# SJTMusicTeam/MusicGeneration

Measured on AMD Instinct MI355X. Metric: training events/sec (whole node), REMI seq_len=2048, higher is better.
Workload: dtype bf16; 1 GPU; cfg2 REMI_EventSeq MusicTransformer V=337 layers=6 d_model=512 seq_len=2048 bf16, fwd+smoothed-CE+bwd+Adam/Noam, dropout 0.2; global_batch=128, per_gpu_batch=128, seq_len=2048, parallelism=dp1, deterministic=True, streams=one stream, whole chip

## Files before the change

### musicgeneration_amd/csrc/rel_attn_bwd.hip

```cpp
#include <type_traits>
#include "rel_attn_common.hpp"

using namespace relattn;

#ifndef MGX_EXPERIMENTS
#define MGX_EXPERIMENTS 0
#endif
namespace {
constexpr int WAVES = 4;
}

__global__ __launch_bounds__(256) void attn_delta_kernel(const uint16_t* __restrict__ ctx,
                                                         const uint16_t* __restrict__ dctx, const float* __restrict__ lse,
                                                         float* __restrict__ delta, float* __restrict__ nlse2,
                                                         float* __restrict__ ndelta, int B, int L, int d) {
    const int heads = d >> 6;
    const long total = (long)B * L * heads * 8;
    const long gid = (long)blockIdx.x * blockDim.x + threadIdx.x;
    if (gid >= total) return;
    const int sub = (int)(gid & 7);
    const long grp = gid >> 3;
    const int i = (int)(grp % L);
    const int hd = (int)((grp / L) % heads);
    const long row = (grp / ((long)L * heads)) * L + i;
// ... 166 lines not shown
#pragma unroll
        for (int ks = 0; ks < 4; ++ks) c = mfma(frag_R(kt, a, hh, ks), qf[ks], c);
        if (MASKED) {
            if (dq == 0) {
#pragma unroll
                for (int r = 0; r < 16; ++r) c[r] = (crow(r, 0) > am) ? -INFINITY : c[r];
            }
            if (pw) {
                const uint32_t pwl = pw >> (4 * hh);
#pragma unroll
                for (int r = 0; r < 16; ++r) c[r] = (pwl & (1u << crow(r, 0))) ? -INFINITY : c[r];
            }
        }
#pragma unroll
        for (int r = 0; r < 16; ++r) c[r] = __builtin_amdgcn_exp2f(__builtin_fmaf(c[r], LOG2E, -lse2));
        f32x16 dp = zero16();
        const char* vt = smem + OFF_VR + cur * TILE_BYTES;
#pragma unroll
        for (int ks = 0; ks < 4; ++ks) dp = mfma(frag_R(vt, a, hh, ks), dof[ks], dp);
#pragma unroll
        for (int r = 0; r < 16; ++r) c[r] = c[r] * (dp[r] - dlt);
        bf16x8 df[2];
#pragma unroll
        for (int ss = 0; ss < 2; ++ss) {
            df[ss] = acc_to_frag(c, ss);
            dq0 = mfma(frag_T_onR(kt, lane, ss, 0), df[ss], dq0);
            dq1 = mfma(frag_T_onR(kt, lane, ss, 1), df[ss], dq1);
        }
#pragma unroll
        for (int ss = 0; ss < 2; ++ss) {
            const u32x4 wv = __builtin_bit_cast(u32x4, df[ss]);
#pragma unroll
            for (int j = 0; j < 4; ++j) {
                const int r0 = 8 * ss + 2 * j;
                *(uint16_t*)(dband + (p ? dwa1[r0] : dwa0[r0])) = (uint16_t)wv[j];
                *(uint16_t*)(dband + (p ? dwa1[r0 + 1] : dwa0[r0 + 1])) = (uint16_t)(wv[j] >> 16);
            }
        }
        wave_lds_fence();
#pragma unroll
        for (int ks = 0; ks < 2; ++ks) {
            const bf16x8 gq = *(const bf16x8*)(dband + a * DB_STRIDE + (p * 32 + 16 * ks + 8 * hh) * 2);
            dq0 = mfma(et[2 * ks], gq, dq0);
            dq1 = mfma(et[2 * ks + 1], gq, dq1);
        }
    };
    const int nmain = anypad ? 0 : Q0;
    auto main_step = [&](int s, auto par_tag) {
        constexpr int PAR = decltype(par_tag)::value;
        const int tn = min(s + 1, ntw - 1);
        const u32x4 kreg = k_tile(tn);
        const u32x4 vreg = v_tile(tn);
        const int dq = q0 - s;
        bf16x8 et[4];
#pragma unroll
        for (int ks = 0; ks < 2; ++ks) { et[2 * ks] = et_frag(dq, ks, 0); et[2 * ks + 1] = et_frag(dq, ks, 1); }
        f32x16 c = zero16();
#pragma unroll
        for (int ks = 0; ks < 4; ++ks) c = mfma(qf[ks], e[ks], c);
        band_put(c, PAR ^ 1);
        wave_lds_fence();
        c = band_get(PAR);
        wave_lds_fence();
#pragma unroll
        for (int ks = 0; ks < 4; ++ks) e[ks] = e_frag(dq - 2, ks);
        __builtin_amdgcn_sched_barrier(0x78F);
        tile_tail(c, dq, PAR, PAR, 0u, std::false_type{}, et);
        *(u32x4*)(smem + OFF_KR + (PAR ^ 1) * TILE_BYTES + st_offR) = kreg;
        *(u32x4*)(smem + OFF_VR + (PAR ^ 1) * TILE_BYTES + st_offR) = vreg;
        __syncthreads();
    };
    int s = 0;
    for (; s < nmain; s += 2) {
        main_step(s, std::integral_constant<int, 0>{});
        main_step(s + 1, std::integral_constant<int, 1>{});
    }

    for (; s < ntw; ++s) {
        const int cur = s & 1;
        const int tn = min(s + 1, ntw - 1);
        const u32x4 kreg = k_tile(tn);
        const u32x4 vreg = v_tile(tn);
        const int dq = q0 - s;
        if (dq >= 0) {
            const uint32_t pw = padword(s);
            bf16x8 et[4];
#pragma unroll
            for (int ks = 0; ks < 2; ++ks) { et[2 * ks] = et_frag(dq, ks, 0); et[2 * ks + 1] = et_frag(dq, ks, 1); }
            if (dq >= 1) {
                f32x16 qe = zero16();
#pragma unroll
                for (int ks = 0; ks < 4; ++ks) qe = mfma(qf[ks], e[ks], qe);
                band_put(qe, cur ^ 1);
            }
            wave_lds_fence();
            f32x16 c = band_get(cur);
            wave_lds_fence();
#pragma unroll
            for (int ks = 0; ks < 4; ++ks) e[ks] = e_frag(dq - 2, ks);
            tile_tail(c, dq, cur, cur, pw, std::true_type{}, et);
        }
        if (s + 1 < ntw) {
            *(u32x4*)(smem + OFF_KR + (cur ^ 1) * TILE_BYTES + st_offR) = kreg;
            *(u32x4*)(smem + OFF_VR + (cur ^ 1) * TILE_BYTES + st_offR) = vreg;
        }
        __syncthreads();
    }
    if (wave_on) store_rows_lds(dqkv + ((size_t)b * L + i0) * ld + hd * 64, ld, dq0, dq1, lane, 0.125f, smem + band_base);
}

#ifndef MGX_DQL_PEEL
#define MGX_DQL_PEEL 0
#endif
#ifndef MGX_DQL_KT
#define MGX_DQL_KT 1
#endif
namespace k1l {
constexpr int OFF_KR = 0;
constexpr int OFF_ET = OFF_KR + 2 * TILE_BYTES;
constexpr int XROW = 72;
constexpr int OFF_X = OFF_ET + 8 * 4096;
constexpr int DB_STRIDE = 144;
constexpr int OFF_DBAND = OFF_X + WAVES * 32 * XROW;
constexpr int LDS_BYTES = OFF_DBAND + WAVES * 32 * DB_STRIDE;
constexpr int DEPTH = 4;
}

__global__ __launch_bounds__(256, 2) void rel_attn_dq_lite_kernel(
    const uint16_t* __restrict__ qkv, const u32x4* __restrict__ EfT, const uint16_t* __restrict__ dst,
    uint16_t* __restrict__ dqkv, int L, int d, int bgroup) {
    using namespace k1l;
    extern __shared__ __attribute__((aligned(256))) char smem[];
    const int tid = threadIdx.x, lane = tid & 63;
    const int w = __builtin_amdgcn_readfirstlane(tid >> 6);
    const int a = lane & 31, hh = lane >> 5;
    const int heads = d >> 6;
    const int nqb = (L + 127) >> 7;
    const int b = (blockIdx.y / nqb) * bgroup + blockIdx.x / heads, hd = blockIdx.x % heads;
    const int qb = nqb - 1 - (blockIdx.y % nqb);
    const int I0 = qb * 128, Q0 = I0 >> 5;
    const int nchunk = L >> 5;
    const bool wave_on = I0 + w * 32 < L;
    const int q0 = wave_on ? Q0 + w : nchunk - 1;
    const int i0 = q0 * 32;
    const int ntw = min(Q0 + 4, nchunk);
    const size_t ld = (size_t)3 * d;
    const uint16_t* qkv_b = qkv + (size_t)b * L * ld;

    const int srow = tid >> 3, sch = tid & 7;
    const int st_offR = MGX_DQL_KT ? imgT_off(srow, sch) : imgR_off(srow, sch);
    const char* k_base = (const char*)(qkv_b + d + hd * 64);
    const uint32_t k_voff = (uint32_t)((srow * ld + sch * 8) * 2);
    const uint32_t tile_bytes = (uint32_t)(32 * ld * 2);
    auto k_tile = [&](int t) { return *(const u32x4*)(k_base + (size_t)min(t, ntw - 1) * tile_bytes + k_voff); };
    const uint32_t tid16 = (uint32_t)tid * 16u, lane16 = (uint32_t)lane * 16u;
    auto e_item = [&](int k) {
        return *(const u32x4*)((const char*)EfT + (size_t)min(max(Q0 - k, 0), nchunk - 1) * 4096 + tid16);
    };
    const size_t ntri = (size_t)nchunk * (nchunk + 1) / 2;
    const size_t row_tiles = ((size_t)b * heads + hd) * ntri + (size_t)q0 * (q0 + 1) / 2;
    const char* ds_row = (const char*)(dst + row_tiles * 1024);
    auto ds_load = [&](int J, int ss) {
        return __builtin_nontemporal_load((const u32x4*)(ds_row + (size_t)min(J, q0) * 2048 + ss * 1024 + lane16));
    };

    u32x4 dsr[DEPTH][2];
#pragma unroll
    for (int j = 0; j < DEPTH; ++j) { dsr[j][0] = ds_load(j, 0); dsr[j][1] = ds_load(j, 1); }
    *(u32x4*)(smem + OFF_KR + st_offR) = k_tile(0);
#pragma unroll
    for (int k = -3; k <= 0; ++k) *(u32x4*)(smem + OFF_ET + (k & 7) * 4096 + tid16) = e_item(k);
    u32x4 kq[2] = {k_tile(1), k_tile(2)}, eq[2] = {e_item(1), e_item(2)};
    for (int o = tid * 16; o < WAVES * 32 * DB_STRIDE; o += 256 * 16) *(u32x4*)(smem + OFF_DBAND + o) = u32x4{0, 0, 0, 0};
    __syncthreads();

    char* xt = smem + OFF_X + w * (32 * XROW);
    char* dband = smem + OFF_DBAND + w * (32 * DB_STRIDE);
    const int xw0 = a * XROW + 8 * hh;
    const int xi = lane & 15, xg = lane >> 4;
    const int xr0 = ((xi >> 2) + 4 * hh) * XROW + 32 * (xg & 1) + 8 * (xi & 3);
    int dwa0[16], dwa1[16];
#pragma unroll
    for (int r = 0; r < 16; ++r) {
        dwa0[r] = crow(r, hh) * DB_STRIDE + (((crow(r, hh) - a) & 63) << 1);
        dwa1[r] = crow(r, hh) * DB_STRIDE + (((crow(r, hh) - a + 32) & 63) << 1);
    }
    f32x16 dq0 = zero16(), dq1 = zero16();

    auto frag_X = [&](int s) {
        bf16x8 out;
#pragma unroll
        for (int jq = 0; jq < 2; ++jq) {
            const bf16x4 t4 = __builtin_amdgcn_ds_read_tr16_b64_v4bf16((lds_bf16x4_ptr)(xt + xr0 + (16 * s + 8 * jq) * XROW));
            out[4 * jq + 0] = t4[0]; out[4 * jq + 1] = t4[1]; out[4 * jq + 2] = t4[2]; out[4 * jq + 3] = t4[3];
        }
        return out;
    };
    auto compute = [&](int p, const char* kt, const char* ec, const u32x4 (&t)[2]) {
#pragma unroll
        for (int ss = 0; ss < 2; ++ss) {
            if (!(MGX_DQL_PEEL & 1)) {
                *(u32x2*)(xt + xw0 + 16 * (2 * ss)) = u32x2{t[ss].x, t[ss].y};
                *(u32x2*)(xt + xw0 + 16 * (2 * ss + 1)) = u32x2{t[ss].z, t[ss].w};
            }
#pragma unroll
            for (int j = 0; j < ((MGX_DQL_PEEL & 2) ? 1 : 4); ++j) {
                const int r0 = 8 * ss + 2 * j;
                *(uint16_t*)(dband + (p ? dwa1[r0] : dwa0[r0])) = (uint16_t)t[ss][j];
                *(uint16_t*)(dband + (p ? dwa1[r0 + 1] : dwa0[r0 + 1])) = (uint16_t)(t[ss][j] >> 16);
            }
        }
        wave_lds_fence();
#pragma unroll
        for (int ss = 0; ss < ((MGX_DQL_PEEL & 4) ? 1 : 2); ++ss) {
            const bf16x8 df = frag_X(ss);
            dq0 = mfma(MGX_DQL_KT ? frag_T(kt, lane, ss, 0) : frag_T_onR(kt, lane, ss, 0), df, dq0);
            dq1 = mfma(MGX_DQL_KT ? frag_T(kt, lane, ss, 1) : frag_T_onR(kt, lane, ss, 1), df, dq1);
        }
#pragma unroll
        for (int ks = 0; ks < ((MGX_DQL_PEEL & 8) ? 1 : 2); ++ks) {
            const bf16x8 gq = *(const bf16x8*)(dband + a * DB_STRIDE + (p * 32 + 16 * ks + 8 * hh) * 2);
            dq0 = mfma(*(const bf16x8*)(ec + (2 * ks) * 1024 + lane16), gq, dq0);
            dq1 = mfma(*(const bf16x8*)(ec + (2 * ks + 1) * 1024 + lane16), gq, dq1);
        }
        wave_lds_fence();
    };
    auto step = [&](int s, auto slot_tag, bool active) {
        constexpr int SLOT = decltype(slot_tag)::value, PAR = SLOT & 1;
        const u32x4 t[2] = {dsr[SLOT][0], dsr[SLOT][1]};
        dsr[SLOT][0] = ds_load(s + DEPTH, 0);
        dsr[SLOT][1] = ds_load(s + DEPTH, 1);
        if (active) compute(PAR, smem + OFF_KR + PAR * TILE_BYTES, smem + OFF_ET + ((s - w) & 7) * 4096, t);
        if (!(MGX_DQL_PEEL & 16)) {
            *(u32x4*)(smem + OFF_KR + (PAR ^ 1) * TILE_BYTES + st_offR) = kq[PAR];
            *(u32x4*)(smem + OFF_ET + ((s + 1) & 7) * 4096 + tid16) = eq[PAR];
            kq[PAR] = k_tile(s + 3);
            eq[PAR] = e_item(s + 3);
        }
        __syncthreads();
    };
    using S0_ = std::integral_constant<int, 0>; using S1_ = std::integral_constant<int, 1>;
    using S2_ = std::integral_constant<int, 2>; using S3_ = std::integral_constant<int, 3>;
    static_assert(DEPTH == 4, "the loops below are unrolled by DEPTH");
    __builtin_amdgcn_s_waitcnt(0x0F70);
    int s = 0;
    for (; s < Q0; s += 4) {
        step(s, S0_{}, true);
        step(s + 1, S1_{}, true);
        step(s + 2, S2_{}, true);
        step(s + 3, S3_{}, true);
    }
    step(s, S0_{}, q0 - s >= 0);
    if (s + 1 < ntw) step(s + 1, S1_{}, q0 - s - 1 >= 0);
    if (s + 2 < ntw) step(s + 2, S2_{}, q0 - s - 2 >= 0);
    if (s + 3 < ntw) step(s + 3, S3_{}, q0 - s - 3 >= 0);
    if (wave_on) store_rows_lds(dqkv + ((size_t)b * L + i0) * ld + hd * 64, ld, dq0, dq1, lane, 0.125f, dband);
}

#ifndef MGX_DKV_PEEL
#define MGX_DKV_PEEL 0
#endif
#ifdef MGX_DKV_STAMP
#define DKV_STAMP(i) do { __builtin_amdgcn_sched_barrier(0); const unsigned long long t_ = __builtin_amdgcn_s_memtime(); \
                          __builtin_amdgcn_sched_barrier(0); if (!MASKED) st_acc[i] += t_ - st_last; st_last = t_; } while (0)
#else
#define DKV_STAMP(i)
#endif
#ifndef MGX_DKV_IMGB
#define MGX_DKV_IMGB 0
#endif
#ifndef MGX_DKV_ONEIMG
#define MGX_DKV_ONEIMG 1
#endif
#ifndef MGX_DKV_WAVES
#define MGX_DKV_WAVES 4
#endif
#if 0
#endif
namespace k2 {
constexpr int KW = MGX_DKV_WAVES;
constexpr int OFF_QR = 0;
constexpr int OFF_QT = OFF_QR + 2 * TILE_BYTES;
constexpr int OFF_OR = OFF_QT + 2 * TILE_BYTES;
constexpr int OFF_OT = OFF_OR + 2 * TILE_BYTES;
constexpr int ST_BYTES = 256 * KW;
constexpr int OFF_ST = OFF_OT + 2 * TILE_BYTES;
constexpr int PATCH_BYTES = 4608;
constexpr int OFF_BAND = KW == 4 ? OFF_ST + 2 * ST_BYTES : 0;
constexpr int OFF_FLAG = KW == 4 ? OFF_BAND + KW * PATCH_BYTES : OFF_ST + 2 * ST_BYTES;
constexpr int LDS_BYTES = OFF_FLAG + 16;
}

template <bool EXPORT_DS>
__global__ __launch_bounds__(64 * k2::KW, 2) void rel_attn_dkv_kernel(
    const uint16_t* __restrict__ qkv, const u32x4* __restrict__ EfA, const uint32_t* __restrict__ padbits,
    const uint16_t* __restrict__ dctx, const float* __restrict__ nlse2 , const float* __restrict__ ndelta ,
    uint16_t* __restrict__ dqkv, uint16_t* __restrict__ dst, int L, int d, int bgroup) {
    using namespace k2;
    extern __shared__ __attribute__((aligned(256))) char smem[];
    const int tid = threadIdx.x, lane = tid & 63;
    const int w = __builtin_amdgcn_readfirstlane(tid >> 6);
    const int bl = lane & 31, hh = lane >> 5;
    const int heads = d >> 6;
    const int nkb = (L + 32 * KW - 1) / (32 * KW);
#ifndef MGX_DKV_XCD
#define MGX_DKV_XCD 0
#endif
    int bh_l = blockIdx.x, kbr = blockIdx.y % nkb;
    if (MGX_DKV_XCD && (gridDim.x & 7) == 0) {
        const int r = kbr * gridDim.x + bh_l, per = gridDim.x >> 3, m = r >> 3;
        kbr = m / per;
        bh_l = (m % per) * 8 + (r & 7);
    }
    const int b = (blockIdx.y / nkb) * bgroup + bh_l / heads, hd = bh_l % heads;
    const int J0 = kbr * 32 * KW;
    const int nchunk = L >> 5;
    const int nT = (L - J0) >> 5;
    const bool wave_on = J0 + w * 32 < L;
    const int wk = wave_on ? w : nT - 1;
    const int j0 = J0 + wk * 32;
    const size_t ld = (size_t)3 * d;
    const uint16_t* qkv_b = qkv + (size_t)b * L * ld;
    const size_t stat_base = ((size_t)b * heads + hd) * L;

    constexpr int NS = 4 / KW;
    const char* q_base = (const char*)(qkv_b + (size_t)J0 * ld + hd * 64);
    const char* o_base = (const char*)(dctx + ((size_t)b * L + J0) * d + hd * 64);
    uint32_t q_voffR[NS], q_voffT[NS], o_voffR[NS], o_voffT[NS];
#pragma unroll
    for (int i = 0; i < NS; ++i) {
        const int slot = tid + 64 * KW * i, srow = slot >> 3, spc = slot & 7;
        const int lcR = spc ^ (MGX_DKV_IMGB ? imgB_swz(srow) : ((srow >> 1) & 7)), lcT = spc ^ (((srow >> 1) & 1) << 2);
        q_voffR[i] = (uint32_t)((srow * ld + lcR * 8) * 2); q_voffT[i] = (uint32_t)((srow * ld + lcT * 8) * 2);
        o_voffR[i] = (uint32_t)((srow * d + lcR * 8) * 2);  o_voffT[i] = (uint32_t)((srow * d + lcT * 8) * 2);
    }
    const uint32_t q_step = (uint32_t)(32 * ld * 2), o_step = (uint32_t)(32 * d * 2);
    const uint32_t lane16 = (uint32_t)lane * 16u;
    auto e_frag = [&](int q, int ks) {
        return __builtin_bit_cast(bf16x8, *(const u32x4*)((const char*)EfA + (size_t)min(max(q, 0), nchunk - 1) * 4096 + ks * 1024 + lane16));
    };
    const uint32_t st_voff = (uint32_t)(((lane & 32) ? (const char*)ndelta - (const char*)nlse2 : 0) + (lane & 31) * 4);
    const char* st_base = (const char*)(nlse2 + stat_base + J0);
    const uint32_t lds_w = lds_addr_of(smem) + w * 1024;
    auto stage = [&](int t, int buf) {
        const int tn = (MGX_DKV_PEEL & 16) ? 0 : min(t, nT - 1);
        const char* qb = q_base + (size_t)tn * q_step;
        const char* ob = o_base + (size_t)tn * o_step;
#pragma unroll
        for (int i = 0; i < NS; ++i) {
            const uint32_t dw = lds_w + KW * 1024 * i + buf * TILE_BYTES;
            dma16(qb, q_voffR[i], dw + OFF_QR);
            if (!MGX_DKV_ONEIMG) dma16(qb, q_voffT[i], dw + OFF_QT);
            dma16(ob, o_voffR[i], dw + OFF_OR);
            if (!MGX_DKV_ONEIMG) dma16(ob, o_voffT[i], dw + OFF_OT);
        }
        dma4(st_base + (size_t)tn * 128, st_voff, lds_addr_of(smem) + OFF_ST + buf * ST_BYTES + w * 256);
    };
    stage(0, 0);
    bf16x8 kf[4], vf[4], e[2][4];
    uint32_t padlane = 0;
    int wgpad = 0;
    {
        const uint16_t* kp = qkv_b + (size_t)(j0 + bl) * ld + d + hd * 64 + hh * 8;
#pragma unroll
        for (int ks = 0; ks < 4; ++ks) {
            kf[ks] = __builtin_bit_cast(bf16x8, *(const u32x4*)(kp + ks * 16));
            vf[ks] = __builtin_bit_cast(bf16x8, *(const u32x4*)(kp + d + ks * 16));
            e[0][ks] = e_frag(0, ks);
            e[1][ks] = e[0][ks];
        }
        if (padbits) {
            const uint32_t pwv = padbits[(size_t)b * nchunk + (j0 >> 5)];
            padlane = (pwv >> bl) & 1u;
            if (tid == 0) *(volatile uint32_t*)(smem + OFF_FLAG) = 0u;
            __syncthreads();
            if (pwv) *(volatile uint32_t*)(smem + OFF_FLAG) = 1u;
            __syncthreads();
            wgpad = __builtin_amdgcn_readfirstlane(*(volatile uint32_t*)(smem + OFF_FLAG));
        }
    }
    asm volatile("s_waitcnt vmcnt(0)" ::: "memory");
    __syncthreads();
    char* band = smem + OFF_BAND + w * PATCH_BYTES;
    uint32_t rd[16];
#pragma unroll
    for (int r = 0; r < 16; ++r) rd[r] = (uint32_t)((hh * 32 + ((crow(r, hh) - bl) & 31)) << 2);
    f32x16 dk0 = zero16(), dk1 = zero16(), dv0 = zero16(), dv1 = zero16();
    char* ds_col = nullptr;
    if (EXPORT_DS) {
        const size_t ntri = (size_t)nchunk * (nchunk + 1) / 2;
        ds_col = (char*)(dst + (((size_t)b * heads + hd) * ntri + (size_t)(j0 >> 5)) * 1024) + lane16;
    }
    auto ds_tile = [&](int t) {
        const size_t I = (size_t)(J0 >> 5) + t;
        return ds_col + (I * (I + 1) / 2) * 2048;
    };

#ifdef MGX_DKV_STAMP
    unsigned long long st_acc[6] = {0, 0, 0, 0, 0, 0}, st_last = 0;
    unsigned st_steps = 0;
    const unsigned long long st_t0 = __builtin_amdgcn_s_memtime(), st_r0 = __builtin_amdgcn_s_memrealtime();
#endif
    auto tile = [&](int dq, int cur, auto par_tag, auto masked_tag, char* dsp, int tnext) {
        constexpr int PAR = decltype(par_tag)::value;
        constexpr bool MASKED = decltype(masked_tag)::value;
        DKV_STAMP(5);
        const char* qr = smem + OFF_QR + cur * TILE_BYTES;
        bf16x8 qa[4];
// ... 224 lines not shown
            for (int ks = 0; ks < 4; ++ks) qa[ks] = frag_R(qr, bl, hh, ks);
            f32x16 qe = zero16();
#pragma unroll
            for (int ks = 0; ks < 4; ++ks) qe = mfma(qa[ks], ef[ks], qe);
#pragma unroll
            for (int r = 0; r < 16; ++r) *(float*)(band + (crow(r, hh) * 32 + bl) * 4) = qe[r];
            wave_lds_fence();
            f32x16 srel;
#pragma unroll
            for (int r = 0; r < 16; ++r) {
                const int ar = crow(r, hh);
                srel[r] = *(const float*)(band + (ar * 32 + ((ar - bl) & 31)) * 4);
            }
            const bool has_up = (u >= 1);
            const char* klo = smem + OFF_KR + (u % KV_SLOTS) * TILE_BYTES;
            const char* vlo = smem + OFF_VR + (u % KV_SLOTS) * TILE_BYTES;
            const char* kup = smem + OFF_KR + ((u + KV_SLOTS - 1) % KV_SLOTS) * TILE_BYTES;
            const char* vup = smem + OFF_VR + ((u + KV_SLOTS - 1) % KV_SLOTS) * TILE_BYTES;
            f32x16 slo = srel, sup = srel;
#pragma unroll
            for (int ks = 0; ks < 4; ++ks) slo = mfma(qa[ks], frag_R(klo, bl, hh, ks), slo);
            if (has_up) {
#pragma unroll
                for (int ks = 0; ks < 4; ++ks) sup = mfma(qa[ks], frag_R(kup, bl, hh, ks), sup);
            }
            bool plo = false, pup = !has_up;
            if (pb) {
                plo = (pb[u] >> bl) & 1u;
                if (has_up) pup = (pb[u - 1] >> bl) & 1u;
            }
            const char* orr = smem + OFF_OR + cur * TILE_BYTES;
            bf16x8 oa[4];
#pragma unroll
            for (int ks = 0; ks < 4; ++ks) oa[ks] = frag_R(orr, bl, hh, ks);
            f32x16 dlo = zero16(), dup = zero16();
#pragma unroll
            for (int ks = 0; ks < 4; ++ks) dlo = mfma(oa[ks], frag_R(vlo, bl, hh, ks), dlo);
            if (has_up) {
#pragma unroll
                for (int ks = 0; ks < 4; ++ks) dup = mfma(oa[ks], frag_R(vup, bl, hh, ks), dup);
            }
            const char* st = smem + OFF_ST + cur * 256;
            f32x16 ds;
#pragma unroll
            for (int g4 = 0; g4 < 4; ++g4) {
                const f32x4 l4 = (MGX_DKV_PEEL & 32) ? f32x4{9.f, 9.f, 9.f, 9.f} : *(const f32x4*)(st + (8 * g4 + 4 * hh) * 4);
                const f32x4 d4 = (MGX_DKV_PEEL & 32) ? f32x4{0.f, 0.f, 0.f, 0.f} : *(const f32x4*)(st + 128 + (8 * g4 + 4 * hh) * 4);
#pragma unroll
                for (int k = 0; k < 4; ++k) {
                    const int r = 4 * g4 + k;
                    const bool lower = (bl <= crow(r, hh));
                    const bool masked = lower ? plo : pup;
                    const float sv = lower ? slo[r] : sup[r];
                    const float dv = lower ? dlo[r] : dup[r];
                    const float p = masked ? 0.f : __builtin_amdgcn_exp2f(__builtin_fmaf(sv, LOG2E, -l4[k]));
                    ds[r] = p * (dv - d4[k]);
                }
            }
            wave_lds_fence();
#pragma unroll
            for (int r = 0; r < 16; ++r) {
                const int ar = crow(r, hh);
                *(float*)(band + (ar * 32 + ((ar - bl) & 31)) * 4) = ds[r];
            }
            wave_lds_fence();
            f32x16 x;
#pragma unroll
            for (int r = 0; r < 16; ++r) x[r] = *(const float*)(band + (crow(r, hh) * 32 + bl) * 4);
            wave_lds_fence();
            const char* qt = smem + OFF_QT + cur * TILE_BYTES;
#pragma unroll
            for (int ss = 0; ss < 2; ++ss) {
                const bf16x8 xf = acc_to_frag(x, ss);
                de0 = mfma(xf, frag_T(qt, lane, ss, 0), de0);
                de1 = mfma(xf, frag_T(qt, lane, ss, 1), de1);
            }
        }
        if (have_next) {
            *(u32x4*)(smem + (half ? OFF_VR : OFF_KR) + ((t + 1) % KV_SLOTS) * TILE_BYTES + st_offR) = kreg;
            if (half == 0) {
                const u32x4 qq = scale8(qreg, 0.125f);
                *(u32x4*)(smem + OFF_QR + (cur ^ 1) * TILE_BYTES + st_offR) = qq;
                *(u32x4*)(smem + OFF_QT + (cur ^ 1) * TILE_BYTES + st_offT) = qq;
            } else {
                *(u32x4*)(smem + OFF_OR + (cur ^ 1) * TILE_BYTES + st_offR) = qreg;
            }
            if (tid < 64) *(float*)(smem + OFF_ST + (cur ^ 1) * 256 + tid * 4) = streg;
        }
        __syncthreads();
    }
    if (wave_on) {
#pragma unroll
        for (int r = 0; r < 16; ++r) {
            const int dl = 32 * cw + crow(r, hh);
            float* row = dEr + (size_t)(L - 1 - dl) * 64;
            atomicAdd(row + bl, de0[r]);
            atomicAdd(row + 32 + bl, de1[r]);
        }
    }
}

#ifndef MGX_DET_PEEL
#define MGX_DET_PEEL 0
#endif
namespace k3t {
#ifndef MGX_DET_STEPS
#define MGX_DET_STEPS 32
#endif
constexpr int DIAGS = 4, RS = 64, STEPS = MGX_DET_STEPS, NW = 5;
constexpr int AROW = 352;
constexpr int OFF_A = 0;
constexpr int OFF_Q = RS * AROW;
constexpr int LDS_BYTES = OFF_Q + 2 * TILE_BYTES;
constexpr int SLOTS = 2;
}

__global__ __launch_bounds__(320, 4) void rel_attn_de_tiles_kernel(
    const uint16_t* __restrict__ qkv, const uint16_t* __restrict__ dst, float* __restrict__ dEr ,
    int bgroup, int ngroups, int wg_per_group, int L, int d,
    long long* __restrict__ det ) {
    using namespace k3t;
    extern __shared__ __attribute__((aligned(16))) char smem[];
    const int tid = threadIdx.x, lane = tid & 63;
    const int w = __builtin_amdgcn_readfirstlane(tid >> 6);
    const int l31 = lane & 31, hh = lane >> 5;
    const int heads = d >> 6, nbh = bgroup * heads;
    const size_t ld = (size_t)3 * d;
    const int nchunk = L >> 5;
    int t = 0, first = 0, ns = 0;
    const bool dealt = ngroups > 0;
    const int xk = dealt ? (int)(blockIdx.x >> 3) : (int)blockIdx.x;
    const int grp = dealt ? (xk / wg_per_group) * 8 + (int)(blockIdx.x & 7) : xk / wg_per_group;
    {
        int rest = xk % wg_per_group;
        const int ntile = (nchunk + DIAGS - 1) / DIAGS;
        for (t = 0; t < ntile; ++t) {
            ns = (L - t * DIAGS * 32 + RS - 1) / RS;
            const int nwg = (nbh * ns + STEPS - 1) / STEPS;
            if (rest < nwg) break;
            rest -= nwg;
        }
        if (t == ntile) return;
        first = rest * STEPS;
    }
    const int total = nbh * ns;
    const int last = min(total, first + STEPS);
    const int c0 = t * DIAGS, d0 = c0 * 32;
    const size_t ntri = (size_t)nchunk * (nchunk + 1) / 2;
    const int qrow = tid >> 3, qch = tid & 7;
    const uint32_t lane16 = (uint32_t)lane * 16u;
    const int wm = w & 3;
    const int sc_lane = hh * 4 * (AROW + 2) - 2 * l31;
    u32x4 areg[SLOTS][2], qreg[2];
    bool a_ok[SLOTS], q_ok[2];
    auto load_tiles = [&](int g) {
        const int bhl = g / ns, i0 = d0 + (g - bhl * ns) * RS;
        const int bh = grp * nbh + bhl;
        const int bb = bh / heads, hd = bh - bb * heads;
        const int I0 = i0 >> 5;
        const char* tp = (const char*)(dst + (size_t)bh * ntri * 1024) + lane16;
#pragma unroll
        for (int k = 0; k < SLOTS; ++k) {
            const int I = I0 + k, J = I - c0 - wm;
            a_ok[k] = I < nchunk && J >= 0;
            const size_t Ic = (size_t)min(I, nchunk - 1), Jc = (size_t)max(J, 0);
            const char* p = tp + (Ic * (Ic + 1) / 2 + min(Jc, Ic)) * 2048;
            areg[k][0] = __builtin_nontemporal_load((const u32x4*)p);
            areg[k][1] = __builtin_nontemporal_load((const u32x4*)(p + 1024));
        }
        const uint16_t* qp = qkv + ((size_t)bb * L + ((MGX_DET_PEEL & 4) ? 0 : i0)) * ld + hd * 64 + (qch & 7) * 8;
#pragma unroll
        for (int i = 0; i < 2; ++i) {
            const int r = (qrow & 31) + 32 * i;
            q_ok[i] = i0 + r < L;
            qreg[i] = *(const u32x4*)(qp + (size_t)min(r, L - 1 - i0) * ld);
        }
    };
    auto store_tiles = [&]() {
        const u32x4 zero = {0, 0, 0, 0};
        if (w < 4) {
#pragma unroll
            for (int k = 0; k < SLOTS; ++k) {
                char* base = smem + OFF_A + k * 32 * AROW + 64 * (wm + 1) + sc_lane;
#pragma unroll
                for (int ss = 0; ss < 2; ++ss) {
                    const u32x4 v = a_ok[k] ? areg[k][ss] : zero;
#pragma unroll
                    for (int j = 0; j < ((MGX_DET_PEEL & 1) ? 1 : 4); ++j) {
                        const int r0 = 8 * ss + 2 * j;
                        *(uint16_t*)(base + crow(r0, 0) * (AROW + 2)) = (uint16_t)v[j];
                        *(uint16_t*)(base + crow(r0 + 1, 0) * (AROW + 2)) = (uint16_t)(v[j] >> 16);
                    }
                }
            }
            char* qt = smem + OFF_Q;
#pragma unroll
            for (int i = 0; i < 2; ++i) {
                const int r = qrow + 32 * i;
                *(u32x4*)(qt + (r >> 5) * TILE_BYTES + imgT_off(r & 31, qch)) = q_ok[i] ? qreg[i] : zero;
            }
        }
    };
    f32x16 de0 = zero16(), de1 = zero16();
    const int fa_i = lane & 15, fa_g = lane >> 4;
    const int fa_off = (fa_i >> 2) * AROW + (32 * w) * 2 + (2 * (fa_g & 1) + ((fa_i & 3) >> 1)) * 16 + 8 * (fa_i & 1) + 8 * hh * AROW;
    auto multiply = [&]() {
        if (MGX_DET_PEEL & 2) return;
        const char* at = smem + OFF_A + fa_off;
        const char* qt = smem + OFF_Q;
#pragma unroll
        for (int ks = 0; ks < 4; ++ks) {
            bf16x8 af;
#pragma unroll
            for (int jq = 0; jq < 2; ++jq) {
                const bf16x4 tq = __builtin_amdgcn_ds_read_tr16_b64_v4bf16((lds_bf16x4_ptr)(at + (16 * ks + 4 * jq) * AROW));
                af[4 * jq + 0] = tq[0]; af[4 * jq + 1] = tq[1]; af[4 * jq + 2] = tq[2]; af[4 * jq + 3] = tq[3];
            }
            const char* qs = qt + (ks >> 1) * TILE_BYTES;
            de0 = mfma(af, frag_Tn(qs, lane, ks & 1, 0), de0);
            de1 = mfma(af, frag_Tn(qs, lane, ks & 1, 1), de1);
        }
    };
    for (int o = tid * 16; o < RS * AROW; o += NW * 64 * 16) *(u32x4*)(smem + OFF_A + o) = u32x4{0, 0, 0, 0};
    __syncthreads();
    if (first < last) {
        load_tiles(first);
        store_tiles();
    }
    __syncthreads();
    for (int g = first; g + 1 < last; ++g) {
        load_tiles(g + 1);
        __builtin_amdgcn_sched_barrier(0);
        multiply();
        __syncthreads();
        store_tiles();
        __syncthreads();
    }
    if (first < last) multiply();
#pragma unroll
    for (int r = 0; r < 16; ++r) {
        const int dl = d0 - 32 + 32 * w + crow(r, hh);
        if ((MGX_DET_PEEL & 8) && de0[r] + de1[r] != 12345.f) continue;
        if (dl >= 0 && dl < L) {
            if (det) {
                long long* drow = det + (size_t)(L - 1 - dl) * 64;
                det_add(drow + l31, 0.125f * de0[r]);
                det_add(drow + 32 + l31, 0.125f * de1[r]);
                continue;
            }
            float* row = dEr + (size_t)(L - 1 - dl) * 64;
            atomicAdd(row + l31, 0.125f * de0[r]);
            atomicAdd(row + 32 + l31, 0.125f * de1[r]);
        }
    }
}

static int bwd_batch_group(int B, int L, int d) {
    const double per_row = (double)L * d * 2 * 5;
    int g = B;
#if MGX_EXPERIMENTS
    static const int forced = [] { const char* e = getenv("MGX_ATTN_BGROUP"); return e ? atoi(e) : 0; }();
    if (forced > 0 && B % forced == 0) return forced;
#endif
    while (g > 1 && (g * per_row > 110e6 || B % g != 0)) --g;
    return g;
}

static size_t ws_stat_bytes(int B, int L, int d) { return (((size_t)B * (d / 64) * L * 4) + 255) / 256 * 256; }
static size_t ws_delta_bytes(int B, int L, int d) { return 3 * ws_stat_bytes(B, L, d); }

static size_t ws_ert_bytes(int L) { return 2 * er_frag_bytes(L); }

extern "C" size_t mgx_rel_attn_bwd_workspace(int B, int L, int d) {
    if (B <= 0 || L <= 0 || d <= 0) return 0;
    const size_t nchunk = (size_t)L / 32;
    return ws_delta_bytes(B, L, d) + ws_ert_bytes(L) + (size_t)B * (d / 64) * (nchunk * (nchunk + 1) / 2) * 2048;
}

extern "C" int mgx_rel_attn_bwd_parts(const uint16_t* qkv, const uint16_t* E, const uint32_t* padbits,
                                      const uint16_t* ctx, const uint16_t* dctx, const float* lse, uint16_t* dqkv,
                                      float* dE, void* workspace, size_t ws_bytes, int B, int L, int d, int M,
                                      int parts, void* stream) {
    MGX_REQUIRE(qkv && E && ctx && dctx && lse && dqkv && dE && workspace, MGX_ERR_NULL, "mgx_rel_attn_bwd: NULL pointer");
    MGX_REQUIRE(B > 0 && L > 0 && d > 0 && d % 64 == 0 && L % 32 == 0 && M >= L, MGX_ERR_SHAPE,
                "mgx_rel_attn_bwd: need d%%64==0, L%%32==0, M>=L (got B=%d L=%d d=%d M=%d)", B, L, d, M);
    MGX_REQUIRE(ws_bytes >= mgx_rel_attn_bwd_workspace(B, L, d) && ((uintptr_t)workspace & 255) == 0, MGX_ERR_SHAPE,
                "mgx_rel_attn_bwd: workspace must be 256-byte aligned and >= mgx_rel_attn_bwd_workspace() = %zu bytes (got %zu)",
                mgx_rel_attn_bwd_workspace(B, L, d), ws_bytes);
    MGX_REQUIRE(!((parts & 2) && (parts & 32)), MGX_ERR_SHAPE, "mgx_rel_attn_bwd: parts 2 and 32 both write dq");
    static const bool attr_once = [] {
        hipFuncSetAttribute((const void*)rel_attn_dq_kernel, hipFuncAttributeMaxDynamicSharedMemorySize, k1::LDS_BYTES);
        hipFuncSetAttribute((const void*)rel_attn_dq_lite_kernel, hipFuncAttributeMaxDynamicSharedMemorySize, k1l::LDS_BYTES);
        hipFuncSetAttribute((const void*)rel_attn_dkv_kernel<true>, hipFuncAttributeMaxDynamicSharedMemorySize, k2::LDS_BYTES);
        hipFuncSetAttribute((const void*)rel_attn_de_kernel, hipFuncAttributeMaxDynamicSharedMemorySize, k3::LDS_BYTES);
        hipFuncSetAttribute((const void*)rel_attn_de_tiles_kernel, hipFuncAttributeMaxDynamicSharedMemorySize, k3t::LDS_BYTES);
        return true;
    }();
    (void)attr_once;
    hipStream_t s = (hipStream_t)stream;
    const int heads = d / 64;
    const uint16_t* Er = E + (size_t)(M - L) * 64;
    float* delta = (float*)workspace;
    float* nlse2 = (float*)((char*)workspace + ws_stat_bytes(B, L, d));
    float* ndelta = (float*)((char*)workspace + 2 * ws_stat_bytes(B, L, d));
    u32x4* EfA = (u32x4*)((char*)workspace + ws_delta_bytes(B, L, d));
    u32x4* EfT = (u32x4*)((char*)EfA + er_frag_bytes(L));
    uint16_t* dst = (uint16_t*)((char*)EfA + ws_ert_bytes(L));
    if (parts & 1) {
        const long total = (long)B * L * heads * 8;
        hipLaunchKernelGGL(attn_delta_kernel, dim3((unsigned)((total + 255) / 256)), dim3(256), 0, s, ctx, dctx, lse, delta, nlse2, ndelta, B, L, d);
        launch_er_frag(Er, EfA, EfT, L, s);
    }
    const int bg = bwd_batch_group(B, L, d);
    MGX_REQUIRE((long)((L + 127) / 128) * (B / bg) <= 65535, MGX_ERR_SHAPE, "mgx_rel_attn_bwd: L/128 * batch groups too large");
    const dim3 gq(bg * heads, ((L + 127) / 128) * (B / bg));
    MGX_REQUIRE(!((parts & 4) && (parts & 64)), MGX_ERR_SHAPE, "mgx_rel_attn_bwd: parts 4 and 64 both write dk / dv and the dS tiles");
#ifndef MGX_DKV64_DEFAULT
#define MGX_DKV64_DEFAULT 1
#endif
    if ((parts & 4) && MGX_DKV64_DEFAULT && L % 128 == 0) {
        const int rc64 = dkv64_launch(qkv, EfA, padbits, dctx, nlse2, ndelta, dqkv, dst, B, L, d, bg, stream);
        if (rc64 != MGX_OK) return rc64;
    } else if (parts & (4 | 64)) {
#if MGX_EXPERIMENTS
        static const int dkv_lds = [] {
            const char* e = getenv("MGX_DKV_LDS");
            const int v = e ? atoi(e) : 0;
            if (v > k2::LDS_BYTES) hipFuncSetAttribute((const void*)rel_attn_dkv_kernel<true>, hipFuncAttributeMaxDynamicSharedMemorySize, v);
            return v > k2::LDS_BYTES ? v : k2::LDS_BYTES;
        }();
#else
        constexpr int dkv_lds = k2::LDS_BYTES;
#endif
        const dim3 gk(bg * heads, ((L + 32 * k2::KW - 1) / (32 * k2::KW)) * (B / bg));
        MGX_REQUIRE(gk.y <= 65535, MGX_ERR_SHAPE, "mgx_rel_attn_bwd: too many key blocks for the grid");
        hipLaunchKernelGGL(rel_attn_dkv_kernel<true>, gk, dim3(64 * k2::KW), dkv_lds, s, qkv, EfA, padbits, dctx, nlse2, ndelta, dqkv, dst, L, d, bg);
    }
    if (parts & 2)
        hipLaunchKernelGGL(rel_attn_dq_lite_kernel, gq, dim3(256), k1l::LDS_BYTES, s, qkv, EfT, dst, dqkv, L, d, bg);
    if (parts & 32)
        hipLaunchKernelGGL(rel_attn_dq_kernel, gq, dim3(256), k1::LDS_BYTES, s, qkv, EfA, EfT, padbits, dctx, lse, delta, dqkv, L, d, bg);
    if (parts & 8) {
#ifndef MGX_DET_BG
#define MGX_DET_BG 1
#endif
        const bool dealt = B % (8 * MGX_DET_BG) == 0;
        const int bgd = dealt ? MGX_DET_BG : bg, ngr = B / bgd;
        long nwg = 0;
        for (int t = 0; t < (L / 32 + k3t::DIAGS - 1) / k3t::DIAGS; ++t)
            nwg += ((long)bgd * heads * ((L - t * k3t::DIAGS * 32 + k3t::RS - 1) / k3t::RS) + k3t::STEPS - 1) / k3t::STEPS;
        const long grid = nwg * ngr;
        MGX_REQUIRE(grid < (1L << 31), MGX_ERR_SHAPE, "mgx_rel_attn_bwd: grid too large");
        int rc;
        long long* det = mgx_det_scratch((size_t)L * 64, stream, &rc);
        if (rc != MGX_OK) return rc;
        hipLaunchKernelGGL(rel_attn_de_tiles_kernel, dim3((unsigned)grid), dim3(64 * k3t::NW), k3t::LDS_BYTES, s, qkv, dst,
                           dE + (size_t)(M - L) * 64, bgd, dealt ? ngr : -ngr, (int)nwg, L, d, det);
        if (det) launch_det_fold(det, dE + (size_t)(M - L) * 64, (size_t)L * 64, 1.f, 1, s);
    }
    if (parts & 16) {
        const dim3 ge(B * heads, ((L >> 5) + k3::W3 - 1) / k3::W3);
        hipLaunchKernelGGL(rel_attn_de_kernel, ge, dim3(64 * k3::W3), k3::LDS_BYTES, s, qkv, Er, padbits, dctx, lse, delta,
                           dE + (size_t)(M - L) * 64, L, d);
    }
    MGX_CHECK_LAUNCH("mgx_rel_attn_bwd");
    return MGX_OK;
}

extern "C" int mgx_rel_attn_bwd(const uint16_t* qkv, const uint16_t* E, const uint32_t* padbits, const uint16_t* ctx,
                                const uint16_t* dctx, const float* lse, uint16_t* dqkv, float* dE, void* workspace,
                                size_t ws_bytes, int B, int L, int d, int M, void* stream) {
    return mgx_rel_attn_bwd_parts(qkv, E, padbits, ctx, dctx, lse, dqkv, dE, workspace, ws_bytes, B, L, d, M, 15, stream);
}
```

### musicgeneration_amd/csrc/rel_attn_common.hpp

```cpp
#pragma once
#include "mgx_common.hpp"

namespace relattn {

constexpr int DH = 64;
constexpr int TILE_BYTES = 32 * DH * 2;
constexpr float LOG2E = 1.4426950408889634f;
constexpr float PAD_NEG = -1.0e9f;

typedef __attribute__((address_space(3))) bf16x4* lds_bf16x4_ptr;
typedef __attribute__((address_space(3))) float* lds_f32_ptr;
typedef __attribute__((address_space(3))) char* lds_char_ptr;
MGX_DEV uint32_t lds_addr_of(const char* p) { return (uint32_t)(uintptr_t)(lds_char_ptr)p; }
MGX_DEV void lds_store_f32(uint32_t addr, float v) { *(lds_f32_ptr)(uintptr_t)addr = v; }

MGX_DEV int crow(int r, int hh) { return (r & 3) + 8 * (r >> 2) + 4 * hh; }

MGX_DEV int imgR_off(int row, int chunk) { return row * 128 + ((chunk ^ ((row >> 1) & 7)) << 4); }
MGX_DEV int imgT_off(int row, int chunk) { return row * 128 + ((chunk ^ (((row >> 1) & 1) << 2)) << 4); }

MGX_DEV bf16x8 frag_R(const char* tile, int row, int hh, int ks) {
    return *(const bf16x8*)(tile + imgR_off(row, 2 * ks + hh));
}

MGX_DEV bf16x8 frag_T(const char* tile, int lane, int s, int ct) {
    const int i = lane & 15, g = lane >> 4, hh = lane >> 5;
    const int rq = i >> 2;
    const int chunk = 4 * ct + 2 * (g & 1) + ((i & 3) >> 1);
    const int byte_in = 8 * (i & 1);
    bf16x8 out;
#pragma unroll
    for (int jq = 0; jq < 2; ++jq) {
        const int row = 16 * s + 8 * jq + 4 * hh + rq;
        const char* p = tile + imgT_off(row, chunk) + byte_in;
        bf16x4 t = __builtin_amdgcn_ds_read_tr16_b64_v4bf16((lds_bf16x4_ptr)p);
        out[4 * jq + 0] = t[0]; out[4 * jq + 1] = t[1]; out[4 * jq + 2] = t[2]; out[4 * jq + 3] = t[3];
    }
    return out;
}

MGX_DEV bf16x8 frag_T_onR(const char* tile, int lane, int s, int ct) {
    const int i = lane & 15, g = lane >> 4, hh = lane >> 5;
    const int rq = i >> 2;
    const int chunk = 4 * ct + 2 * (g & 1) + ((i & 3) >> 1);
    const int byte_in = 8 * (i & 1);
    bf16x8 out;
#pragma unroll
    for (int jq = 0; jq < 2; ++jq) {
        const int row = 16 * s + 8 * jq + 4 * hh + rq;
        bf16x4 t = __builtin_amdgcn_ds_read_tr16_b64_v4bf16((lds_bf16x4_ptr)(tile + imgR_off(row, chunk) + byte_in));
        out[4 * jq + 0] = t[0]; out[4 * jq + 1] = t[1]; out[4 * jq + 2] = t[2]; out[4 * jq + 3] = t[3];
    }
    return out;
}

MGX_DEV int imgB_swz(int row) { return (((row >> 1) & 1) << 2) | (((row >> 3) & 1) << 1) | ((row >> 2) & 1); }
MGX_DEV int imgB_off(int row, int chunk) { return row * 128 + ((chunk ^ imgB_swz(row)) << 4); }
MGX_DEV bf16x8 frag_B(const char* tile, int row, int hh, int ks) {
    return *(const bf16x8*)(tile + imgB_off(row, 2 * ks + hh));
}
MGX_DEV bf16x8 frag_T_onB(const char* tile, int lane, int s, int ct) {
    const int i = lane & 15, g = lane >> 4, hh = lane >> 5;
    const int rq = i >> 2;
    const int chunk = 4 * ct + 2 * (g & 1) + ((i & 3) >> 1);
    const int byte_in = 8 * (i & 1);
    bf16x8 out;
#pragma unroll
    for (int jq = 0; jq < 2; ++jq) {
        const int row = 16 * s + 8 * jq + 4 * hh + rq;
        bf16x4 t = __builtin_amdgcn_ds_read_tr16_b64_v4bf16((lds_bf16x4_ptr)(tile + imgB_off(row, chunk) + byte_in));
        out[4 * jq + 0] = t[0]; out[4 * jq + 1] = t[1]; out[4 * jq + 2] = t[2]; out[4 * jq + 3] = t[3];
    }
    return out;
}

MGX_DEV u32x4 scale8(const u32x4& raw, float sc) {
    float f[8];
    unpack8(raw, f);
#pragma unroll
    for (int k = 0; k < 8; ++k) f[k] *= sc;
    return pack8(f);
}

MGX_DEV bf16x8 acc_to_frag(const f32x16& c, int s) {
    u32x4 w;
    w.x = pack_bf16x2(c[8 * s + 0], c[8 * s + 1]);
    w.y = pack_bf16x2(c[8 * s + 2], c[8 * s + 3]);
    w.z = pack_bf16x2(c[8 * s + 4], c[8 * s + 5]);
    w.w = pack_bf16x2(c[8 * s + 6], c[8 * s + 7]);
    return __builtin_bit_cast(bf16x8, w);
}

MGX_DEV f32x16 mfma(const bf16x8& a, const bf16x8& b, const f32x16& c) {
    return __builtin_amdgcn_mfma_f32_32x32x16_bf16(a, b, c, 0, 0, 0);
}

MGX_DEV f32x16 zero16() {
    f32x16 z;
#pragma unroll
    for (int r = 0; r < 16; ++r) z[r] = 0.f;
    return z;
}

constexpr int BAND_STRIDE = 272;
constexpr int BAND_BYTES = 32 * BAND_STRIDE;
MGX_DEV int band_off(int row, int col) { return row * BAND_STRIDE + col * 4; }
constexpr int BAND_REGION = 16 * BAND_STRIDE;
MGX_DEV int band_rowoff(int a) { return ((a & 3) | ((a >> 3) << 2)) * BAND_STRIDE + ((a >> 2) & 1) * BAND_REGION; }
MGX_DEV void band_store(char* band, const int (&wa0)[16], const int (&wa1)[16], int odd, const f32x16& v) {
    if (odd) {
#pragma unroll
        for (int r = 0; r < 16; ++r) *(float*)(band + wa1[r]) = v[r];
    } else {
#pragma unroll
        for (int r = 0; r < 16; ++r) *(float*)(band + wa0[r]) = v[r];
    }
}

MGX_DEV void dma16(const char* sbase , uint32_t voff, uint32_t lds_wave_base) {
    asm volatile("s_mov_b32 m0, %2\n\ts_nop 0\n\tglobal_load_lds_dwordx4 %1, %0" ::"s"(sbase), "v"(voff), "s"(lds_wave_base) : "memory", "m0");
}
MGX_DEV void dma4(const char* sbase , uint32_t voff, uint32_t lds_wave_base) {
    asm volatile("s_mov_b32 m0, %2\n\ts_nop 0\n\tglobal_load_lds_dword %1, %0" ::"s"(sbase), "v"(voff), "s"(lds_wave_base) : "memory", "m0");
}

MGX_DEV void wave_lds_fence() {
    __builtin_amdgcn_fence(__ATOMIC_RELEASE, "wavefront");
    __builtin_amdgcn_wave_barrier();
    __builtin_amdgcn_fence(__ATOMIC_ACQUIRE, "wavefront");
}

MGX_DEV void store_rows_lds(uint16_t* dst, size_t row_stride, const f32x16& t0, const f32x16& t1, int lane, float sc,
                            char* patch) {
    const int x = lane & 31, hh = lane >> 5;
    wave_lds_fence();
#pragma unroll
    for (int g4 = 0; g4 < 4; ++g4) {
        *(u32x2*)(patch + x * 144 + (8 * g4 + 4 * hh) * 2) =
            u32x2{pack_bf16x2(t0[4 * g4] * sc, t0[4 * g4 + 1] * sc), pack_bf16x2(t0[4 * g4 + 2] * sc, t0[4 * g4 + 3] * sc)};
        *(u32x2*)(patch + x * 144 + (32 + 8 * g4 + 4 * hh) * 2) =
            u32x2{pack_bf16x2(t1[4 * g4] * sc, t1[4 * g4 + 1] * sc), pack_bf16x2(t1[4 * g4 + 2] * sc, t1[4 * g4 + 3] * sc)};
    }
    wave_lds_fence();
    const int rr = lane >> 3, ch = lane & 7;
#pragma unroll
    for (int i = 0; i < 4; ++i) {
        const int row = rr + 8 * i;
        *(u32x4*)(dst + (size_t)row * row_stride + ch * 8) = *(const u32x4*)(patch + row * 144 + ch * 16);
    }
    wave_lds_fence();
}

inline size_t er_frag_bytes(int L) { return (((size_t)L * 64 * 2) + 255) / 256 * 256; }

static __global__ __launch_bounds__(256) void er_frag_kernel(const uint16_t* __restrict__ Er, u32x4* __restrict__ EfA,
                                                             u32x4* __restrict__ EfT, int L) {
    const int n = (L >> 5) * 4 * 64;
    const int gid = blockIdx.x * blockDim.x + threadIdx.x;
    if (gid < n) {
        const int lane = gid & 63, ks = (gid >> 6) & 3, q = gid >> 8;
        const int delta = 32 * q + (lane & 31);
        EfA[gid] = *(const u32x4*)(Er + (size_t)(L - 1 - delta) * 64 + 16 * ks + 8 * (lane >> 5));
    } else if (gid < 2 * n && EfT) {
        const int g = gid - n;
        const int lane = g & 63, ct = (g >> 6) & 1, ks = (g >> 7) & 1, q = g >> 8;
        const int col = 32 * ct + (lane & 31);
        uint16_t v[8];
#pragma unroll
        for (int j = 0; j < 8; ++j) {
            const int delta = 32 * q + 16 * ks + 8 * (lane >> 5) + j;
            v[j] = Er[(size_t)(L - 1 - delta) * 64 + col];
        }
        u32x4 o;
        o.x = v[0] | ((uint32_t)v[1] << 16); o.y = v[2] | ((uint32_t)v[3] << 16);
        o.z = v[4] | ((uint32_t)v[5] << 16); o.w = v[6] | ((uint32_t)v[7] << 16);
        EfT[g] = o;
    }
}

static inline void launch_er_frag(const uint16_t* Er, u32x4* EfA, u32x4* EfT, int L, hipStream_t s) {
    const int n = (L >> 5) * 4 * 64 * (EfT ? 2 : 1);
    hipLaunchKernelGGL(er_frag_kernel, dim3((n + 255) / 256), dim3(256), 0, s, Er, EfA, EfT, L);
}

int dkv64_launch(const uint16_t* qkv, const void* EfA, const uint32_t* padbits, const uint16_t* dctx, const float* nlse2,
                 const float* ndelta, uint16_t* dqkv, uint16_t* dst, int B, int L, int d, int bg, void* stream);
int fwd64a_launch(const uint16_t* qkv, const void* Ef, const uint32_t* padbits, uint16_t* ctx, float* lse, int B, int L, int d, int bg,
                  void* stream);
int fwd64_launch(const uint16_t* qkv, const void* EfA, const uint32_t* padbits, uint16_t* ctx, float* lse, int B, int L, int d,
                 void* stream);
int fwdpp_launch(const uint16_t* qkv, const void* EfA, const uint32_t* padbits, uint16_t* ctx, float* lse, int B, int L, int d,
                 void* stream);

}
```

Before: 5.208 million events/s.

## Use inline-asm global loads with counted vmcnt waits in dQ and dST kernels

Replaces the compiler-generated global loads in the dQ backward kernel and the dS-tile transpose kernel with inline-asm global_load_dwordx4 calls. Explicit s_waitcnt vmcnt(N) waits let each wave consume only the loads that have already landed instead of draining all outstanding memory. The dQ kernel's K/E prefetch queue deepens from 2 to 4 slots, and its step now splits into LDS parking and MFMA products so the next loads can be issued in between. The hand-counted wait values depend on exact request ordering, so any change in that order risks reading registers before the data arrives. The deeper queue also raises register pressure.

```diff
diff --git a/musicgeneration_amd/csrc/rel_attn_bwd.hip b/musicgeneration_amd/csrc/rel_attn_bwd.hip
--- a/musicgeneration_amd/csrc/rel_attn_bwd.hip
+++ b/musicgeneration_amd/csrc/rel_attn_bwd.hip
@@ -342,17 +342,18 @@
     const char* k_base = (const char*)(qkv_b + d + hd * 64);
     const uint32_t k_voff = (uint32_t)((srow * ld + sch * 8) * 2);
     const uint32_t tile_bytes = (uint32_t)(32 * ld * 2);
-    auto k_tile = [&](int t) { return *(const u32x4*)(k_base + (size_t)min(t, ntw - 1) * tile_bytes + k_voff); };
+    auto k_addr = [&](int t) { return k_base + (size_t)min(t, ntw - 1) * tile_bytes + k_voff; };
+    auto k_tile = [&](int t) { return *(const u32x4*)k_addr(t); };
     const uint32_t tid16 = (uint32_t)tid * 16u, lane16 = (uint32_t)lane * 16u;
-    auto e_item = [&](int k) {
-        return *(const u32x4*)((const char*)EfT + (size_t)min(max(Q0 - k, 0), nchunk - 1) * 4096 + tid16);
-    };
+    auto e_addr = [&](int k) {
+        return (const char*)EfT + (size_t)min(max(Q0 - k, 0), nchunk - 1) * 4096 + tid16;
+    };
+    auto e_item = [&](int k) { return *(const u32x4*)e_addr(k); };
     const size_t ntri = (size_t)nchunk * (nchunk + 1) / 2;
     const size_t row_tiles = ((size_t)b * heads + hd) * ntri + (size_t)q0 * (q0 + 1) / 2;
     const char* ds_row = (const char*)(dst + row_tiles * 1024);
-    auto ds_load = [&](int J, int ss) {
-        return __builtin_nontemporal_load((const u32x4*)(ds_row + (size_t)min(J, q0) * 2048 + ss * 1024 + lane16));
-    };
+    auto ds_addr = [&](int J) { return ds_row + (size_t)min(J, q0) * 2048 + lane16; };
+    auto ds_load = [&](int J, int ss) { return __builtin_nontemporal_load((const u32x4*)(ds_addr(J) + ss * 1024)); };
 
     u32x4 dsr[DEPTH][2];
 #pragma unroll
@@ -360,7 +361,9 @@
     *(u32x4*)(smem + OFF_KR + st_offR) = k_tile(0);
 #pragma unroll
     for (int k = -3; k <= 0; ++k) *(u32x4*)(smem + OFF_ET + (k & 7) * 4096 + tid16) = e_item(k);
-    u32x4 kq[2] = {k_tile(1), k_tile(2)}, eq[2] = {e_item(1), e_item(2)};
+    u32x4 kq[DEPTH], eq[DEPTH];
+#pragma unroll
+    for (int k = 1; k < DEPTH; ++k) { kq[k] = k_tile(k); eq[k] = e_item(k); }
     for (int o = tid * 16; o < WAVES * 32 * DB_STRIDE; o += 256 * 16) *(u32x4*)(smem + OFF_DBAND + o) = u32x4{0, 0, 0, 0};
     __syncthreads();
 
@@ -386,7 +389,7 @@
         }
         return out;
     };
-    auto compute = [&](int p, const char* kt, const char* ec, const u32x4 (&t)[2]) {
+    auto park = [&](int p, const u32x4 (&t)[2]) {
 #pragma unroll
         for (int ss = 0; ss < 2; ++ss) {
             if (!(MGX_DQL_PEEL & 1)) {
@@ -401,6 +404,8 @@
             }
         }
         wave_lds_fence();
+    };
+    auto products = [&](int p, const char* kt, const char* ec) {
 #pragma unroll
         for (int ss = 0; ss < ((MGX_DQL_PEEL & 4) ? 1 : 2); ++ss) {
             const bf16x8 df = frag_X(ss);
@@ -415,35 +420,45 @@
         }
         wave_lds_fence();
     };
-    auto step = [&](int s, auto slot_tag, bool active) {
-        constexpr int SLOT = decltype(slot_tag)::value, PAR = SLOT & 1;
-        const u32x4 t[2] = {dsr[SLOT][0], dsr[SLOT][1]};
-        dsr[SLOT][0] = ds_load(s + DEPTH, 0);
-        dsr[SLOT][1] = ds_load(s + DEPTH, 1);
-        if (active) compute(PAR, smem + OFF_KR + PAR * TILE_BYTES, smem + OFF_ET + ((s - w) & 7) * 4096, t);
-        if (!(MGX_DQL_PEEL & 16)) {
-            *(u32x4*)(smem + OFF_KR + (PAR ^ 1) * TILE_BYTES + st_offR) = kq[PAR];
-            *(u32x4*)(smem + OFF_ET + ((s + 1) & 7) * 4096 + tid16) = eq[PAR];
-            kq[PAR] = k_tile(s + 3);
-            eq[PAR] = e_item(s + 3);
+    constexpr int RQ = (MGX_DQL_PEEL & 16) ? 2 : 4;
+    auto step = [&](int s, auto slot_tag, auto tail_tag, bool active) {
+        constexpr int SLOT = decltype(slot_tag)::value, PAR = SLOT & 1, NEXT = (SLOT + 1) & 3, TAIL = decltype(tail_tag)::value;
+        if (TAIL < 0 && RQ == 4) {
+            gload16<0>(kq[SLOT], k_addr(s + DEPTH));
+            gload16<0>(eq[SLOT], e_addr(s + DEPTH));
+        }
+        landed<TAIL < 0 ? 4 * RQ - 2 : (3 - TAIL) * RQ>(dsr[SLOT][0], dsr[SLOT][1]);
+        if (active) park(PAR, dsr[SLOT]);
+        if (TAIL < 0) {
+            const char* dp = ds_addr(s + DEPTH);
+            gload16_nt<0>(dsr[SLOT][0], dp);
+            gload16_nt<1024>(dsr[SLOT][1], dp);
+        }
+        if (active) products(PAR, smem + OFF_KR + PAR * TILE_BYTES, smem + OFF_ET + ((s - w) & 7) * 4096);
+        if (RQ == 4 && TAIL < 3) {
+            landed<TAIL < 0 ? 14 : 10 - 4 * TAIL>(kq[NEXT], eq[NEXT]);
+            *(u32x4*)(smem + OFF_KR + (PAR ^ 1) * TILE_BYTES + st_offR) = kq[NEXT];
+            *(u32x4*)(smem + OFF_ET + ((s + 1) & 7) * 4096 + tid16) = eq[NEXT];
         }
         __syncthreads();
     };
     using S0_ = std::integral_constant<int, 0>; using S1_ = std::integral_constant<int, 1>;
     using S2_ = std::integral_constant<int, 2>; using S3_ = std::integral_constant<int, 3>;
+    using LOOP_ = std::integral_constant<int, -1>;
     static_assert(DEPTH == 4, "the loops below are unrolled by DEPTH");
     __builtin_amdgcn_s_waitcnt(0x0F70);
     int s = 0;
     for (; s < Q0; s += 4) {
-        step(s, S0_{}, true);
-        step(s + 1, S1_{}, true);
-        step(s + 2, S2_{}, true);
-        step(s + 3, S3_{}, true);
-    }
-    step(s, S0_{}, q0 - s >= 0);
-    if (s + 1 < ntw) step(s + 1, S1_{}, q0 - s - 1 >= 0);
-    if (s + 2 < ntw) step(s + 2, S2_{}, q0 - s - 2 >= 0);
-    if (s + 3 < ntw) step(s + 3, S3_{}, q0 - s - 3 >= 0);
+        step(s, S0_{}, LOOP_{}, true);
+        step(s + 1, S1_{}, LOOP_{}, true);
+        step(s + 2, S2_{}, LOOP_{}, true);
+        step(s + 3, S3_{}, LOOP_{}, true);
+    }
+    step(s, S0_{}, S0_{}, q0 - s >= 0);
+    if (s + 1 < ntw) step(s + 1, S1_{}, S1_{}, q0 - s - 1 >= 0);
+    if (s + 2 < ntw) step(s + 2, S2_{}, S2_{}, q0 - s - 2 >= 0);
+    if (s + 3 < ntw) step(s + 3, S3_{}, S3_{}, q0 - s - 3 >= 0);
+    asm volatile("s_waitcnt vmcnt(0)" ::: "memory");
     if (wave_on) store_rows_lds(dqkv + ((size_t)b * L + i0) * ld + hd * 64, ld, dq0, dq1, lane, 0.125f, dband);
 }
 
@@ -974,6 +989,8 @@
     const int wm = w & 3;
     const int sc_lane = hh * 4 * (AROW + 2) - 2 * l31;
     u32x4 areg[SLOTS][2], qreg[2];
+    const char* ap[SLOTS];
+    const uint16_t* qp2[2];
     bool a_ok[SLOTS], q_ok[2];
     auto load_tiles = [&](int g) {
         const int bhl = g / ns, i0 = d0 + (g - bhl * ns) * RS;
@@ -986,21 +1003,29 @@
             const int I = I0 + k, J = I - c0 - wm;
             a_ok[k] = I < nchunk && J >= 0;
             const size_t Ic = (size_t)min(I, nchunk - 1), Jc = (size_t)max(J, 0);
-            const char* p = tp + (Ic * (Ic + 1) / 2 + min(Jc, Ic)) * 2048;
-            areg[k][0] = __builtin_nontemporal_load((const u32x4*)p);
-            areg[k][1] = __builtin_nontemporal_load((const u32x4*)(p + 1024));
+            ap[k] = tp + (Ic * (Ic + 1) / 2 + min(Jc, Ic)) * 2048;
         }
         const uint16_t* qp = qkv + ((size_t)bb * L + ((MGX_DET_PEEL & 4) ? 0 : i0)) * ld + hd * 64 + (qch & 7) * 8;
 #pragma unroll
         for (int i = 0; i < 2; ++i) {
             const int r = (qrow & 31) + 32 * i;
             q_ok[i] = i0 + r < L;
-            qreg[i] = *(const u32x4*)(qp + (size_t)min(r, L - 1 - i0) * ld);
+            qp2[i] = qp + (size_t)min(r, L - 1 - i0) * ld;
+        }
+        if (w < 4) {
+            gload16_nt<0>(areg[0][0], ap[0]);
+            gload16_nt<1024>(areg[0][1], ap[0]);
+            gload16_nt<0>(areg[1][0], ap[1]);
+            gload16_nt<1024>(areg[1][1], ap[1]);
+            gload16<0>(qreg[0], qp2[0]);
+            gload16<0>(qreg[1], qp2[1]);
         }
     };
     auto store_tiles = [&]() {
         const u32x4 zero = {0, 0, 0, 0};
         if (w < 4) {
+            static_assert(SLOTS == 2, "the counted waits below are written for six requests per step");
+            landed<5>(areg[0][0]); landed<4>(areg[0][1]); landed<3>(areg[1][0]); landed<2>(areg[1][1]);
 #pragma unroll
             for (int k = 0; k < SLOTS; ++k) {
                 char* base = smem + OFF_A + k * 32 * AROW + 64 * (wm + 1) + sc_lane;
@@ -1016,6 +1041,7 @@
                 }
             }
             char* qt = smem + OFF_Q;
+            landed<1>(qreg[0]); landed<0>(qreg[1]);
 #pragma unroll
             for (int i = 0; i < 2; ++i) {
                 const int r = qrow + 32 * i;
@@ -1052,7 +1078,6 @@
     __syncthreads();
     for (int g = first; g + 1 < last; ++g) {
         load_tiles(g + 1);
-        __builtin_amdgcn_sched_barrier(0);
         multiply();
         __syncthreads();
         store_tiles();
diff --git a/musicgeneration_amd/csrc/rel_attn_common.hpp b/musicgeneration_amd/csrc/rel_attn_common.hpp
--- a/musicgeneration_amd/csrc/rel_attn_common.hpp
+++ b/musicgeneration_amd/csrc/rel_attn_common.hpp
@@ -123,6 +123,15 @@
 MGX_DEV void dma4(const char* sbase , uint32_t voff, uint32_t lds_wave_base) {
     asm volatile("s_mov_b32 m0, %2\n\ts_nop 0\n\tglobal_load_lds_dword %1, %0" ::"s"(sbase), "v"(voff), "s"(lds_wave_base) : "memory", "m0");
 }
+
+template <int OFF> MGX_DEV void gload16(u32x4& dst, const void* p) {
+    asm volatile("global_load_dwordx4 %0, %1, off offset:%2" : "=&v"(dst) : "v"(p), "n"(OFF));
+}
+template <int OFF> MGX_DEV void gload16_nt(u32x4& dst, const void* p) {
+    asm volatile("global_load_dwordx4 %0, %1, off offset:%2 nt" : "=&v"(dst) : "v"(p), "n"(OFF));
+}
+template <int N> MGX_DEV void landed(u32x4& r) { asm volatile("s_waitcnt vmcnt(%1)" : "+v"(r) : "n"(N)); }
+template <int N> MGX_DEV void landed(u32x4& r0, u32x4& r1) { asm volatile("s_waitcnt vmcnt(%2)" : "+v"(r0), "+v"(r1) : "n"(N)); }
 
 MGX_DEV void wave_lds_fence() {
     __builtin_amdgcn_fence(__ATOMIC_RELEASE, "wavefront");
```

Result: no change. 5.184 million events/s (-0.5%).
